# laprade117/interactive-unet

Measured on AMD Instinct MI355X. Metric: voxels/sec (train step + full-volume predict) on 128^3 chunks, higher is better.
Workload: dtype bf16

## Files before the change

interactive-unet_amd/csrc/common.h:

```cpp
#pragma once
#include <hip/hip_runtime.h>
#include <stdint.h>
#include <cstdio>
#include <cstdlib>
#include <type_traits>
#include "../../include/iunet.h"
#include "launchers.h"

typedef _Float16 f16;
typedef __bf16 bf16;
typedef _Float16 f16x8 __attribute__((ext_vector_type(8)));
typedef _Float16 f16x4 __attribute__((ext_vector_type(4)));
typedef _Float16 f16x2 __attribute__((ext_vector_type(2)));
typedef __bf16 bf16x8 __attribute__((ext_vector_type(8)));
typedef float f32x4 __attribute__((ext_vector_type(4)));
typedef unsigned int u32x4 __attribute__((ext_vector_type(4)));

struct TView {
  void* ptr;
  long long sample_stride;
  int planes;
};

template <typename T> struct Vec8;
// ... 262 lines not shown
  a = __builtin_amdgcn_cvt_pk_fp8_f32(c[2], c[3], a, true);
  int b = __builtin_amdgcn_cvt_pk_fp8_f32(c[4], c[5], 0, false);
  b = __builtin_amdgcn_cvt_pk_fp8_f32(c[6], c[7], b, true);
  return u32x2_t{(unsigned)a, (unsigned)b};
}
__device__ __forceinline__ u32x2_t x2m_hi8(const f16x8 hi);
template <bool CLAMPED = false>
__device__ __forceinline__ void x2m_split8(const float (&r)[8], f16x8& hi, f16x8& lo, u32x2_t& lo8, u32x2_t& hi8) {
  typedef short s16x2 __attribute__((ext_vector_type(2)));
  float res[8];
#pragma unroll
  for (int j = 0; j < 8; ++j) {
    const float v = CLAMPED ? r[j] : fminf(fmaxf(r[j], -65504.f), 65504.f);
    const f16 h = (f16)v;
    res[j] = v - (float)h;
    hi[j] = h; lo[j] = (f16)res[j];
  }
  s16x2 a = s16x2{0, 0}, b = s16x2{0, 0};
  a = __builtin_amdgcn_cvt_scalef32_pk_fp8_f32(a, res[0], res[1], 0.0625f, false);
  a = __builtin_amdgcn_cvt_scalef32_pk_fp8_f32(a, res[2], res[3], 0.0625f, true);
  b = __builtin_amdgcn_cvt_scalef32_pk_fp8_f32(b, res[4], res[5], 0.0625f, false);
  b = __builtin_amdgcn_cvt_scalef32_pk_fp8_f32(b, res[6], res[7], 0.0625f, true);
  lo8 = u32x2_t{__builtin_bit_cast(unsigned, a), __builtin_bit_cast(unsigned, b)};
  hi8 = x2m_hi8(hi);
}
__device__ __forceinline__ float x2_load_in(const void* p, long long off, int dt) {
  switch (dt) {
    case 0: return ((const float*)p)[off];
    case 1: return (float)((const f16*)p)[off];
    case 2: return __fdiv_rn((float)((const unsigned char*)p)[off], 255.0f);
    default: return (float)((const bf16*)p)[off];
  }
}
__device__ __forceinline__ void x2m_pool_keys(const f16x8 hi, const u32x2_t lo8, unsigned (&k)[8]) {
  const u32x4 hb = __builtin_bit_cast(u32x4, hi);
  unsigned hf[4], lf[2];
#pragma unroll
  for (int d = 0; d < 4; ++d) hf[d] = hb[d] ^ (((hb[d] >> 15) & 0x00010001u) * 0x7fffu + 0x80008000u);
#pragma unroll
  for (int e = 0; e < 2; ++e) {
    const unsigned t = (lo8[e] >> 7) & 0x01010101u;
    lf[e] = lo8[e] ^ (((t << 7) - t) + 0x80808080u);
  }
#pragma unroll
  for (int j = 0; j < 8; ++j)
    k[j] = __builtin_amdgcn_perm(hf[j >> 1], lf[j >> 2], 0x0c000000u | ((5u + 2u * (j & 1)) << 16) | ((4u + 2u * (j & 1)) << 8) | (unsigned)(j & 3));
}
__device__ __forceinline__ void x2m_pool_unkeys(const unsigned (&k)[8], f16x8& hi, u32x2_t& lo8) {
  u32x4 hb;
#pragma unroll
  for (int d = 0; d < 4; ++d) {
    const unsigned f = __builtin_amdgcn_perm(k[2 * d + 1], k[2 * d], 0x06050201u);
    hb[d] = f ^ (0xffffffffu - ((f >> 15) & 0x00010001u) * 0x7fffu);
  }
#pragma unroll
  for (int e = 0; e < 2; ++e) {
    const unsigned t0 = __builtin_amdgcn_perm(k[4 * e + 1], k[4 * e], 0x0c0c0400u), t1 = __builtin_amdgcn_perm(k[4 * e + 3], k[4 * e + 2], 0x0c0c0400u);
    const unsigned f = __builtin_amdgcn_perm(t1, t0, 0x05040100u);
    const unsigned t = (f >> 7) & 0x01010101u;
    lo8[e] = f ^ (0xffffffffu - ((t << 7) - t));
  }
  hi = __builtin_bit_cast(f16x8, hb);
}
__device__ __forceinline__ unsigned lane_xor1(unsigned v) {
  return (unsigned)__builtin_amdgcn_update_dpp(0, (int)v, 0xB1, 0xF, 0xF, false);
}
// ... 37 lines not shown
```

interactive-unet_amd/csrc/loss_terms.h:

```cpp
#pragma once
#include "common.h"

namespace {

__device__ __forceinline__ float load_t(const void* p, long long off, int dt) {
  return dt == 0 ? ((const float*)p)[off] : (float)((const f16*)p)[off];
}

__device__ __forceinline__ float block_sum_256(float v, float* red ) {
  v = wave_sum(v);
  __syncthreads();
  if ((threadIdx.x & 63) == 0) red[threadIdx.x >> 6] = v;
  __syncthreads();
  return red[0] + red[1] + red[2] + red[3];
}

template <int NV>
__device__ __forceinline__ void block_reduce_store(const float (&vals)[NV], float* lds, float* out) {
  const int lane = threadIdx.x & 63, wave = threadIdx.x >> 6;
#pragma unroll
  for (int i = 0; i < NV; ++i) {
    const float v = wave_sum(vals[i]);
    if (lane == 0) lds[wave * NV + i] = v;
  }
  __syncthreads();
  for (int i = threadIdx.x; i < NV; i += 256) out[i] = lds[i] + lds[NV + i] + lds[2 * NV + i] + lds[3 * NV + i];
}

template <int NCLS>
__device__ __forceinline__ void loss_sums(const float (&l)[NCLS], const void* target, const void* weight, int tdtype, int n,
                                          long long vox, long long v, float (&acc)[NCLS][8]) {
  float mx = l[0];
#pragma unroll
  for (int c = 1; c < NCLS; ++c) mx = fmaxf(mx, l[c]);
  float e[NCLS], s = 0.f;
#pragma unroll
  for (int c = 0; c < NCLS; ++c) { e[c] = __expf(l[c] - mx); s += e[c]; }
  const float inv = 1.f / s;
#pragma unroll
  for (int c = 0; c < NCLS; ++c) {
    const float pr = e[c] * inv;
    const long long to = ((long long)n * NCLS + c) * vox + v;
    const float y = load_t(target, to, tdtype);
    const float w = weight ? load_t(weight, to, tdtype) : 1.f;
    const float ry = rintf(y), rp = rintf(pr);
    acc[c][0] += w; acc[c][1] += w * y; acc[c][2] += w * pr; acc[c][3] += w * y * pr;
    acc[c][4] += w * y * __logf(pr + 1e-12f);
    acc[c][5] += w * ry; acc[c][6] += w * rp; acc[c][7] += w * ry * rp;
  }
}

template <int NCLS>
__device__ __forceinline__ void loss_grad(const float (&l)[NCLS], const void* target, const void* weight, int tdtype, const float* coef,
                                          int n, long long vox, long long v, float lscale, float (&dl)[NCLS], float (&accb)[NCLS]) {
  float mx = l[0];
#pragma unroll
  for (int c = 1; c < NCLS; ++c) mx = fmaxf(mx, l[c]);
  float e[NCLS], s = 0.f;
#pragma unroll
  for (int c = 0; c < NCLS; ++c) { e[c] = __expf(l[c] - mx); s += e[c]; }
  const float inv = 1.f / s;
  float g[NCLS], dot = 0.f;
#pragma unroll
  for (int c = 0; c < NCLS; ++c) {
    const float pr = e[c] * inv;
    const long long to = ((long long)n * NCLS + c) * vox + v;
    const float y = load_t(target, to, tdtype);
    const float w = weight ? load_t(weight, to, tdtype) : 1.f;
    g[c] = w * (coef[c * 3] + coef[c * 3 + 1] * y) - coef[c * 3 + 2] * w * y / (pr + 1e-12f);
    e[c] = pr;
    dot += g[c] * pr;
  }
#pragma unroll
  for (int c = 0; c < NCLS; ++c) { dl[c] = e[c] * (g[c] - dot) * lscale; accb[c] += dl[c]; }
}

}
```

interactive-unet_amd/csrc/pointwise.hip:

```cpp
#include "common.h"
#include "head_out.h"

namespace {

struct FirstConvParams {
  const void* x;
  long long sN, sC, sD, sH, sW;
  int in_dtype;
  void* y; long long y_sstride;
  const void* w;
  const float* bias;
  float* stats;
  int N, D, H, W, Cin, Cout, nd, relu;
  int out8;
};

__device__ __forceinline__ float load_in(const void* p, long long off, int dt) {
  switch (dt) {
    case 0: return ((const float*)p)[off];
    case 1: return (float)((const f16*)p)[off];
    case 2: return (float)((const unsigned char*)p)[off] / 255.0f;
    default: return (float)((const bf16*)p)[off];
  }
}

template <typename T, int ND, int CIN>
__global__ __launch_bounds__(256) void first_conv_kernel(FirstConvParams p) {
  using V8 = typename Vec8<T>::type;
  constexpr int TZ = ND == 3 ? 4 : 1, TY = ND == 3 ? 8 : 16, TX = ND == 3 ? 16 : 32, PADZ = ND == 3 ? 1 : 0;
  constexpr int PZ = TZ + 2 * PADZ, PY = TY + 2, PX = TX + 2, NPIX = PZ * PY * PX;
  constexpr int TAPS = ND == 3 ? 27 : 9, KK = TAPS * CIN, KS = (KK + 31) / 32;
  constexpr int FX = TX / 16, NI = 8;
  __shared__ T xs[CIN * NPIX];
  __shared__ float red[4 * 4 * 8 * 2];
  const int tid = threadIdx.x, lane = tid & 63, wave = tid >> 6, l15 = lane & 15, q = lane >> 4;
  const int tilesZ = (p.D + TZ - 1) / TZ, tilesY = (p.H + TY - 1) / TY, tilesX = (p.W + TX - 1) / TX;
  const int tps = tilesZ * tilesY * tilesX;
  const int tile = blockIdx.x, n = tile / tps;
  int trem = tile - n * tps;
  const int tz_i = trem / (tilesY * tilesX);
  trem -= tz_i * tilesY * tilesX;
  const int ty_i = trem / tilesX, tx_i = trem - ty_i * tilesX;
  const int z0 = tz_i * TZ, y0 = ty_i * TY, x0 = tx_i * TX;
  const int cob = blockIdx.y;
  for (int it = tid; it < NPIX * CIN; it += 256) {
    const int c = it / NPIX, pix = it - c * NPIX;
    const int px = pix % PX, t2 = pix / PX, py = t2 % PY, pz = t2 / PY;
    const int gz = z0 + pz - PADZ, gy = y0 + py - 1, gx = x0 + px - 1;
    float v = 0.f;
    if ((unsigned)gz < (unsigned)p.D && (unsigned)gy < (unsigned)p.H && (unsigned)gx < (unsigned)p.W)
      v = load_in(p.x, n * p.sN + c * p.sC + gz * p.sD + gy * p.sH + gx * p.sW, p.in_dtype);
    xs[it] = from_f32<T>(v);
  }
  V8 a[KS][2];
  const V8* wp = (const V8*)p.w + (long long)cob * KS * 2 * 64 + lane;
#pragma unroll
  for (int ks = 0; ks < KS; ++ks) { a[ks][0] = wp[(ks * 2 + 0) * 64]; a[ks][1] = wp[(ks * 2 + 1) * 64]; }
  int koff[KS][8];
#pragma unroll
  for (int ks = 0; ks < KS; ++ks)
#pragma unroll
    for (int j = 0; j < 8; ++j) {
      const int k = 32 * ks + 8 * q + j;
      const int kc = k < KK ? k : 0;
      const int tap = kc / CIN, c = kc % CIN;
      const int dz = ND == 3 ? tap / 9 : 0, dy = (tap / 3) % 3, dx = tap % 3;
      koff[ks][j] = c * NPIX + (dz * PY + dy) * PX + dx;
    }
  __syncthreads();
  T* yout = (T*)p.y + (long long)n * p.y_sstride;
  const long long plane_stride = (long long)p.D * p.H * p.W * 8;
  float bias[8], s_sum[8], s_sq[8];
#pragma unroll
  for (int j = 0; j < 8; ++j) { bias[j] = p.bias ? p.bias[cob * 32 + 8 * q + j] : 0.f; s_sum[j] = 0.f; s_sq[j] = 0.f; }
#pragma unroll
  for (int nf = 0; nf < NI; ++nf) {
    const int f = wave * NI + nf;
    const int xh = f % FX, row = f / FX, fy = row % TY, fz = row / TY;
    const int base = (fz * PY + fy) * PX + xh * 16 + l15;
    f32x4 acc0 = f32x4{0, 0, 0, 0}, acc1 = f32x4{0, 0, 0, 0};
#pragma unroll
    for (int ks = 0; ks < KS; ++ks) {
      V8 b;
#pragma unroll
      for (int j = 0; j < 8; ++j) b[j] = xs[base + koff[ks][j]];
      acc0 = mfma16<T>(a[ks][0], b, acc0);
      acc1 = mfma16<T>(a[ks][1], b, acc1);
    }
    const int gz = z0 + fz, gy = y0 + fy, gx = x0 + xh * 16 + l15;
    const bool ok = gz < p.D && gy < p.H && gx < p.W;
    float vals[8];
#pragma unroll
    for (int j = 0; j < 4; ++j) { vals[j] = acc0[j]; vals[4 + j] = acc1[j]; }
    if (p.stats && ok) {
#pragma unroll
      for (int j = 0; j < 8; ++j) { s_sum[j] += vals[j]; s_sq[j] += vals[j] * vals[j]; }
    }
    V8 o;
#pragma unroll
    for (int j = 0; j < 8; ++j) {
      float r = vals[j] + bias[j];
      if (p.relu) r = fmaxf(r, 0.f);
      o[j] = from_f32<T>(r);
    }
    if (ok) {
      if (!p.out8) *(V8*)(yout + (long long)(cob * 4 + q) * plane_stride + (((long long)gz * p.H + gy) * p.W + gx) * 8) = o;
      else e4m3_store8<T>((unsigned char*)p.y + (long long)n * p.y_sstride, cob * 4 + q, ((long long)gz * p.H + gy) * p.W + gx,
// ... 685 lines not shown
```

interactive-unet_amd/csrc/train_misc.hip:

```cpp
#include "common.h"

namespace {


struct ConvTDgradParams {
  const void* dy; long long dy_ss;
  void* dx; long long dx_ss;
  const void* wpk;
  int N, D, H, W, Cin, Cout;
};

template <typename T, int ND>
__global__ __launch_bounds__(256) void convT_dgrad_kernel(ConvTDgradParams p) {
  using V8 = V8T<T>;
  constexpr int NPOS = ND == 3 ? 8 : 4;
  const int lane = threadIdx.x & 63, wave = threadIdx.x >> 6;
  const int l15 = lane & 15, q = lane >> 4;
  const int xg = (p.W + 15) / 16;
  const long long rows = (long long)p.D * p.H * xg;
  const long long wid = (long long)blockIdx.x * 4 + wave;
  if (wid >= rows * p.N) return;
  const int n = (int)(wid / rows);
  const long long r = wid - n * rows;
  const int xb = (int)(r % xg), y = (int)((r / xg) % p.H), z = (int)(r / ((long long)xg * p.H));
// ... 305 lines not shown
  const long long per_b4 = (long long)Cin * Cout * npos / 4;
  const int col4 = threadIdx.x & 15, grp = threadIdx.x >> 4;
  const long long j4 = (long long)blockIdx.x * 16 + col4;
  const f32x4* slab4 = (const f32x4*)slab;
  f32x4 s = f32x4{0.f, 0.f, 0.f, 0.f};
  for (int b = grp; b < nb; b += 16) s += slab4[b * per_b4 + j4];
  red[grp][col4] = s;
  __syncthreads();
  if (grp != 0) return;
#pragma unroll
  for (int g = 1; g < 16; ++g) s += red[g][col4];
  const int ncob = Cout / 32;
#pragma unroll
  for (int k = 0; k < 4; ++k) {
    const long long j = j4 * 4 + k;
    const int c = (int)(j & 31), r = (int)((j >> 5) & 31);
    long long t = j >> 10;
    const int pos = (int)(t % npos); t /= npos;
    const int cob = (int)(t % ncob), cib = (int)(t / ncob);
    dW[((long long)(cib * 32 + r) * Cout + cob * 32 + c) * npos + pos] = s[k];
  }
}

struct FirstWgradParams {
  const void* x; long long sN, sC, sD, sH, sW; int in_dtype;
  const void* dy; long long dy_ss;
  const void* yraw; long long y_ss;
  const float* mean; const float* invstd; const float* coef; const float* scale; const float* shift;
  float* slab;
  int N, D, H, W, Cin, Cout;
  int tilesZ, tilesY, tilesX;
};

__device__ __forceinline__ float load_in2(const void* p, long long off, int dt) {
  switch (dt) {
    case 0: return ((const float*)p)[off];
    case 1: return (float)((const f16*)p)[off];
    case 2: return (float)((const unsigned char*)p)[off] / 255.0f;
    default: return (float)((const bf16*)p)[off];
  }
}

template <typename T, int ND, int CIN>
__global__ __launch_bounds__(256, 2) void first_wgrad_kernel(FirstWgradParams p) {
  using V8 = V8T<T>;
  constexpr int TZ = ND == 3 ? 4 : 1, TY = ND == 3 ? 8 : 16, TX = ND == 3 ? 16 : 32, PADZ = ND == 3 ? 1 : 0;
  constexpr int PZ = TZ + 2 * PADZ, PY = TY + 2, PX = TX + 2, NPIX = PZ * PY * PX, NVOX = TZ * TY * TX;
  constexpr int TAPS = ND == 3 ? 27 : 9, KK = TAPS * CIN, NT = (KK + 15) / 16, KKP = NT * 16;
  constexpr int FX = TX / 16, NKS = NVOX / 32;
  constexpr int PLANE_Y = NVOX * 16 + 64;
  constexpr int XS_BYTES = ((CIN * NPIX * 2 + 255) / 256) * 256;
  extern __shared__ __attribute__((aligned(256))) unsigned char smem[];
  T* xs = (T*)smem;
  unsigned char* dys = smem + XS_BYTES;
  __shared__ __attribute__((aligned(16))) float par[7 * 32];
  if (p.yraw != nullptr && threadIdx.x < 7 * 32) {
    const int k = threadIdx.x >> 5, c = blockIdx.y * 32 + (threadIdx.x & 31);
    par[threadIdx.x] = k == 0 ? p.scale[c] : k == 1 ? p.shift[c] : k == 2 ? p.mean[c] : k == 3 ? p.invstd[c] : p.coef[c * 3 + (k - 4)];
  }
  const unsigned lds_y = (unsigned)(size_t)(__attribute__((address_space(3))) unsigned char*)dys;
  const int tid = threadIdx.x, lane = tid & 63;
  const int wave = __builtin_amdgcn_readfirstlane(tid >> 6);
  const int g = lane >> 4, i16 = lane & 15, q = i16 >> 2, pp = i16 & 3, gh = g >> 1, gl = g & 1;
  const int cob = blockIdx.y;
  const unsigned laneY = lds_y + (pp >> 1) * PLANE_Y + (pp & 1) * 8 + (gh * 16 + gl * 8 + q) * 16;
  int col_off[NT];
#pragma unroll
  for (int ct = 0; ct < NT; ++ct) {
    const int kk = ct * 16 + i16, kc = kk < KK ? kk : 0;
    const int tap = kc / CIN, c = kc % CIN;
    const int dz = ND == 3 ? tap / 9 : 0, dy_ = (tap / 3) % 3, dx = tap % 3;
    col_off[ct] = c * NPIX + (dz * PY + dy_) * PX + dx;
  }
  f32x4 acc[2][NT];
#pragma unroll
  for (int t = 0; t < 2; ++t)
#pragma unroll
    for (int ct = 0; ct < NT; ++ct) acc[t][ct] = f32x4{0, 0, 0, 0};
  const int tps = p.tilesZ * p.tilesY * p.tilesX, ntiles = tps * p.N;
  const long long plane = (long long)p.D * p.H * p.W * 8;
  constexpr int XIT = (NPIX * CIN + 255) / 256, YIT = NVOX * 4 / 256;
  float xr[XIT];
  u32x4 yr[YIT], yw[YIT];
  unsigned oky = 0;
  auto load_tile = [&](int tile) {
    oky = 0;
    const int n = tile / tps;
    int trem = tile - n * tps;
    const int tz_i = trem / (p.tilesY * p.tilesX);
    trem -= tz_i * p.tilesY * p.tilesX;
    const int ty_i = trem / p.tilesX, tx_i = trem - ty_i * p.tilesX;
    const int z0 = tz_i * TZ, y0 = ty_i * TY, x0 = tx_i * TX;
#pragma unroll
    for (int k = 0; k < XIT; ++k) {
      const int it = tid + k * 256;
      const int c = it / NPIX, pix = it - c * NPIX;
      const int px = pix % PX, t2 = pix / PX, py = t2 % PY, pz = t2 / PY;
      const int gz = z0 + pz - PADZ, gy = y0 + py - 1, gx = x0 + px - 1;
      float v = 0.f;
      if (it < NPIX * CIN && (unsigned)gz < (unsigned)p.D && (unsigned)gy < (unsigned)p.H && (unsigned)gx < (unsigned)p.W)
        v = load_in2(p.x, n * p.sN + c * p.sC + gz * p.sD + gy * p.sH + gx * p.sW, p.in_dtype);
      xr[k] = v;
    }
    const T* dyin = (const T*)p.dy + (long long)n * p.dy_ss + (long long)cob * 4 * plane;
#pragma unroll
    for (int it = 0; it < YIT; ++it) {
      const int idx = tid + it * 256, pl = idx / NVOX, pix = idx - pl * NVOX;
      const int px = pix % TX, t2 = pix / TX, py = t2 % TY, pz = t2 / TY;
      const int gz = z0 + pz, gy = y0 + py, gx = x0 + px;
      u32x4 v = u32x4{0u, 0u, 0u, 0u};
      if (gz < p.D && gy < p.H && gx < p.W) v = *(const u32x4*)(dyin + pl * plane + (((long long)gz * p.H + gy) * p.W + gx) * 8);
      yr[it] = v;
      oky |= (gz < p.D && gy < p.H && gx < p.W) ? (1u << it) : 0u;
      if (p.yraw != nullptr) {
        u32x4 w = u32x4{0u, 0u, 0u, 0u};
        if (gz < p.D && gy < p.H && gx < p.W)
          w = *(const u32x4*)((const T*)p.yraw + (long long)n * p.y_ss + (long long)(cob * 4 + pl) * plane + (((long long)gz * p.H + gy) * p.W + gx) * 8);
        yw[it] = w;
      }
    }
  };
  auto commit_tile = [&]() {
#pragma unroll
    for (int k = 0; k < XIT; ++k) {
      const int it = tid + k * 256;
      if (it < NPIX * CIN) xs[it] = from_f32<T>(xr[k]);
    }
#pragma unroll
    for (int it = 0; it < YIT; ++it) {
      const int idx = tid + it * 256, pl = idx / NVOX, pix = idx - pl * NVOX;
      u32x4 v = yr[it];
      if (p.yraw != nullptr && ((oky >> it) & 1u)) {
        const V8 g = __builtin_bit_cast(V8, v), yy = __builtin_bit_cast(V8, yw[it]);
        V8 o;
        const f32x4* pp = (const f32x4*)(par + pl * 8);
        float cs[7][8];
#pragma unroll
        for (int k = 0; k < 7; ++k) {
          const f32x4 lo = pp[k * 8], hi = pp[k * 8 + 1];
#pragma unroll
          for (int j = 0; j < 4; ++j) { cs[k][j] = lo[j]; cs[k][4 + j] = hi[j]; }
        }
#pragma unroll
        for (int j = 0; j < 8; ++j) {
          const float yv = to_f32<T>(yy[j]);
          const float zv = to_f32<T>(from_f32<T>(fmaf(cs[0][j], yv, cs[1][j])));
          const float d = zv > 0.f ? to_f32<T>(g[j]) : 0.f;
          const float xh = (yv - cs[2][j]) * cs[3][j];
          o[j] = from_f32<T>(cs[4][j] * (d - cs[5][j] - xh * cs[6][j]));
        }
        v = __builtin_bit_cast(u32x4, o);
      }
      *(u32x4*)(dys + pl * PLANE_Y + pix * 16) = v;
    }
  };
  if ((int)blockIdx.x < ntiles) load_tile(blockIdx.x);
  for (int tile = blockIdx.x; tile < ntiles; tile += gridDim.x) {
    __syncthreads();
    commit_tile();
    __syncthreads();
    if (tile + (int)gridDim.x < ntiles) load_tile(tile + gridDim.x);
    for (int ks = wave; ks < NKS; ks += 4) {
      const int f = 2 * ks + gh;
      const int xh = f % FX, row = f / FX, fy = row % TY, fz = row / TY;
      const int vbase = (fz * PY + fy) * PX + xh * 16 + gl * 8;
      const V8 a0 = tr_frag2<T>(laneY + (unsigned)(2 * ks * 256), 64);
      const V8 a1 = tr_frag2<T>(laneY + (unsigned)(2 * ks * 256) + 2 * PLANE_Y, 64);
#pragma unroll
      for (int ct = 0; ct < NT; ++ct) {
        V8 b;
#pragma unroll
        for (int j = 0; j < 8; ++j) b[j] = xs[vbase + j + col_off[ct]];
        acc[0][ct] = mfma16<T>(a0, b, acc[0][ct]);
        acc[1][ct] = mfma16<T>(a1, b, acc[1][ct]);
      }
    }
  }
  __syncthreads();
  float* red = (float*)smem;
#pragma unroll
  for (int t = 0; t < 2; ++t)
#pragma unroll
    for (int ct = 0; ct < NT; ++ct)
#pragma unroll
      for (int j = 0; j < 4; ++j) red[(wave * 32 + t * 16 + 4 * g + j) * KKP + ct * 16 + i16] = acc[t][ct][j];
  __syncthreads();
  float* slab = p.slab + ((long long)blockIdx.x * p.Cout + cob * 32) * KKP;
// ... 198 lines not shown
```

interactive-unet_amd/csrc/train_pointwise.hip:

```cpp
#include "common.h"
#include "loss_terms.h"

namespace {


__global__ __launch_bounds__(1024) void bn_finalize_kernel(const float* __restrict__ slab, int nparts, int C, double count,
                                                           const float* __restrict__ gamma, const float* __restrict__ beta,
                                                           float* running_mean, float* running_var, float momentum,
                                                           float eps, float* scale, float* shift, float* mean_o,
                                                           float* invstd_o) {
  const int c = blockIdx.x, nt = (int)blockDim.x, nw = nt >> 6;
  double s = 0.0, s2 = 0.0;
  for (int p = threadIdx.x; p < nparts; p += nt) {
    const float2 v = *(const float2*)(slab + ((long long)p * C + c) * 2);
    s += (double)v.x; s2 += (double)v.y;
  }
  __shared__ double red[2][16];
#pragma unroll
  for (int o = 32; o > 0; o >>= 1) { s += __shfl_xor(s, o); s2 += __shfl_xor(s2, o); }
  if ((threadIdx.x & 63) == 0) { red[0][threadIdx.x >> 6] = s; red[1][threadIdx.x >> 6] = s2; }
  __syncthreads();
  if (threadIdx.x == 0) {
    double g0[4], g1[4];
    for (int g = 0; g < nw / 4; ++g) {
// ... 447 lines not shown
      const float base = add_skip ? to_f32<T>(o[j]) : 0.f;
      o[j] = from_f32<T>(base + (best[j] == s ? to_f32<T>(g[j]) : 0.f));
    }
    *(V8T<T>*)(dz + n * dz_ss + off[s]) = o;
  }
}

struct HeadLossParams {
  const void* x; long long x_ss; int planes;
  const float* w; const float* bias;
  const void* target; const void* weight; int tdtype;
  float* slab;
  const float* coef;
  void* dx; long long dx_ss;
  float* dwslab;
  float loss_scale;
  const float* loss_scale_dev;
  int N; long long vox;
  const float* in_scale; const float* in_shift;
  int pss;
};

template <typename T>
__device__ __forceinline__ V8T<T> head_act(const HeadLossParams& p, V8T<T> v, int pl, int n) {
  if (p.in_scale == nullptr) return v;
  V8T<T> o;
#pragma unroll
  for (int j = 0; j < 8; ++j)
    o[j] = from_f32<T>(fmaxf(fmaf(p.in_scale[n * p.pss + pl * 8 + j], to_f32<T>(v[j]), p.in_shift[n * p.pss + pl * 8 + j]), 0.f));
  return o;
}

#define HEAD_FWD_ITER 8
template <typename T, int NCLS>
__global__ __launch_bounds__(256) void head_loss_fwd_kernel(HeadLossParams p) {
  const int n = blockIdx.y;
  float acc[NCLS][8];
#pragma unroll
  for (int c = 0; c < NCLS; ++c)
#pragma unroll
    for (int k = 0; k < 8; ++k) acc[c][k] = 0.f;
  for (int it = 0; it < HEAD_FWD_ITER; ++it) {
    const long long v = ((long long)blockIdx.x * HEAD_FWD_ITER + it) * 256 + threadIdx.x;
    if (v >= p.vox) break;
    const T* xin = (const T*)p.x + n * p.x_ss + v * 8;
    float l[NCLS];
#pragma unroll
    for (int c = 0; c < NCLS; ++c) l[c] = p.bias[c];
    for (int pl = 0; pl < p.planes; ++pl) {
      const V8T<T> xv = head_act<T>(p, *(const V8T<T>*)(xin + (long long)pl * p.vox * 8), pl, n);
#pragma unroll
      for (int j = 0; j < 8; ++j) {
        const float a = to_f32<T>(xv[j]);
#pragma unroll
        for (int c = 0; c < NCLS; ++c) l[c] = fmaf(a, p.w[c * p.planes * 8 + pl * 8 + j], l[c]);
      }
    }
    loss_sums<NCLS>(l, p.target, p.weight, p.tdtype, n, p.vox, v, acc);
  }
  __shared__ float red[4 * NCLS * 8];
  const long long part = (long long)n * gridDim.x + blockIdx.x;
  float vals[NCLS * 8];
#pragma unroll
  for (int c = 0; c < NCLS; ++c)
#pragma unroll
    for (int k = 0; k < 8; ++k) vals[c * 8 + k] = acc[c][k];
  block_reduce_store<NCLS * 8>(vals, red, p.slab + part * NCLS * 8);
}

__global__ __launch_bounds__(256) void loss_finalize_kernel(const float* __restrict__ slab, int nparts, int ncls, int kind,
                                                            int has_weight, double nvox_total, float* out ,
                                                            float* coef ) {
  __shared__ double sums[10][8];
  __shared__ double red[256];
  const int items = ncls * 8, groups = 256 / items, t = threadIdx.x;
  double s = 0.0;
  if (t < groups * items) {
    const long long total = (long long)nparts * items;
    long long e = t;
    for (; e + 3LL * groups * items < total; e += 4LL * groups * items) {
      const float a = slab[e], b = slab[e + (long long)groups * items], c = slab[e + 2LL * groups * items],
                  d = slab[e + 3LL * groups * items];
      s += (double)a; s += (double)b; s += (double)c; s += (double)d;
    }
    for (; e < total; e += (long long)groups * items) s += (double)slab[e];
  }
  red[t] = s;
  __syncthreads();
  if (t < items) {
    double a = 0.0;
    for (int g = 0; g < groups; ++g) a += red[g * items + t];
    sums[t >> 3][t & 7] = a;
  }
  __syncthreads();
  if (threadIdx.x != 0) return;
  const double eps = 1e-12;
  const bool use_ce = (kind == 0 || kind >= 4);
  const int base = kind >= 4 ? kind - 3 : kind;
  double loss = 0.0, dice_r = 0.0, iou_r = 0.0, mcc_r = 0.0;
  const double G = (double)ncls;
  for (int c = 0; c < ncls; ++c) {
    const double cnt = has_weight ? sums[c][0] : nvox_total;
    const double tp = sums[c][3] / cnt, fp = (sums[c][2] - sums[c][3]) / cnt, fn = (sums[c][1] - sums[c][3]) / cnt;
    const double tn = (sums[c][0] - sums[c][1] - sums[c][2] + sums[c][3]) / cnt;
    double s_tp = 0, s_tn = 0, s_fp = 0, s_fn = 0, score = 0;
    if (base == 1) {
      const double num = 2 * tp + eps, den = 2 * tp + fp + fn + eps;
      score = num / den; s_tp = (2 * den - 2 * num) / (den * den); s_fp = -num / (den * den); s_fn = s_fp;
    } else if (base == 2) {
      const double num = tp + eps, den = tp + fp + fn + eps;
      score = num / den; s_tp = (den - num) / (den * den); s_fp = -num / (den * den); s_fn = s_fp;
    } else if (base == 3) {
      const double a = tp + fp, b = tp + fn, cc = tn + fp, d = tn + fn;
      const double root = sqrt(a * b * cc * d), num = tp * tn - fp * fn + eps, den = root + eps;
      score = num / den;
      const double half = 0.5 / root;
      const double r_tp = half * (b * cc * d + a * cc * d), r_tn = half * (a * b * d + a * b * cc);
      const double r_fp = half * (b * cc * d + a * b * d), r_fn = half * (a * cc * d + a * b * cc);
      s_tp = (tn * den - num * r_tp) / (den * den); s_tn = (tp * den - num * r_tn) / (den * den);
      s_fp = (-fn * den - num * r_fp) / (den * den); s_fn = (-fp * den - num * r_fn) / (den * den);
    }
    if (base != 0) loss += (1.0 - score) / G;
    if (use_ce) loss += (-sums[c][4] / cnt) / G;
    const double k = -1.0 / (G * cnt);
    coef[c * 3 + 0] = (float)(k * (s_fp - s_tn));
    coef[c * 3 + 1] = (float)(k * ((s_tp - s_fn) - (s_fp - s_tn)));
// ... 543 lines not shown
    const float mn = b1 * mv + (1.f - b1) * gr;
    const float vn = b2 * vv + (1.f - b2) * gr * gr;
    mv = mn; vv = vn;
    const float denom = sqrtf(vn) / bc2_sqrt + eps;
    pn -= (lr / bc1) * (mn / denom);
    pv = pn;
  };
  const long long i = ((long long)blockIdx.x * 256 + threadIdx.x) * 4;
  if (i + 3 < n) {
    float4 pv = *(float4*)(p + i), mv = *(float4*)(m + i), vv = *(float4*)(v + i);
    const float4 gv = *(const float4*)(g + i);
    one(pv.x, gv.x, mv.x, vv.x); one(pv.y, gv.y, mv.y, vv.y); one(pv.z, gv.z, mv.z, vv.z); one(pv.w, gv.w, mv.w, vv.w);
    *(float4*)(p + i) = pv; *(float4*)(m + i) = mv; *(float4*)(v + i) = vv;
  } else {
    for (long long k = i; k < n; ++k) one(p[k], g[k], m[k], v[k]);
  }
}
__global__ void head_grad_scatter_kernel(const float* __restrict__ t, float* __restrict__ dw, float* __restrict__ db, int ncls, int C0) {
  const int i = blockIdx.x * blockDim.x + threadIdx.x;
  if (i < ncls * C0) {
    const int c = i / C0, ch = i - c * C0;
    dw[i] = t[((ch >> 3) * ncls + c) * 8 + (ch & 7)];
  } else if (i < ncls * C0 + ncls) {
    db[i - ncls * C0] = t[i];
  }
}

}

#define DT_OK(dt) IUNET_REQUIRE((dt) == 0 || (dt) == 1, "dtype must be 0 (f16) or 1 (bf16), got %d", (dt))

int iunet_loss_finalize_launch(const float* slab, int nparts, int ncls, int kind, int has_weight, double nvox_total, float* out4,
                               float* coef, hipStream_t stream) {
  hipLaunchKernelGGL(loss_finalize_kernel, dim3(1), dim3(256), 0, stream, slab, nparts, ncls, kind, has_weight, nvox_total, out4, coef);
  IUNET_CHECK_HIP(hipGetLastError());
  return IUNET_OK;
}

static const int BN_BWD_PER_BLOCK = 2048;
static const int BN_POOL_PER_BLOCK = 8192;
static int norm_pool_chunks(int nd, long long ovox) {
  const int per_block = BN_POOL_PER_BLOCK / (nd == 3 ? 8 : 4);
  return (int)((ovox + per_block - 1) / per_block);
}

static int norm_relu_fwd_launch(int dtype, const void* y, long long y_ss, void* z, long long z_ss, const void* scale, const void* shift, int C,
                                int N, long long vox, int pss, void* stream) {
  const dim3 grid((unsigned)((vox + 511) / 512), C / 8, N);
  iunet_dispatch(dtype, 2, false, [&](auto t, auto, auto) {
    using T = decltype(t);
    hipLaunchKernelGGL(bn_relu_fwd_kernel<T>, grid, dim3(256), 0, (hipStream_t)stream, (const T*)y, y_ss, (T*)z, z_ss, (const float*)scale,
                       (const float*)shift, C / 8, vox, pss);
  });
  IUNET_CHECK_HIP(hipGetLastError());
  return IUNET_OK;
}
static int norm_relu_pool_fwd_launch(int dtype, int nd, const void* y, long long y_ss, void* z, long long z_ss, void* pooled, long long p_ss,
                                     const void* scale, const void* shift, int C, int N, int Do, int Ho, int Wo, int pss, void* stream) {
  const long long ovox = (long long)Do * Ho * Wo;
  const dim3 grid((unsigned)((ovox + 255) / 256), C / 8, N);
  iunet_dispatch(dtype, nd, false, [&](auto t, auto ndc, auto) {
    using T = decltype(t);
    hipLaunchKernelGGL((bn_relu_pool_fwd_kernel<T, ndc.value>), grid, dim3(256), 0, (hipStream_t)stream, (const T*)y, y_ss, (T*)z, z_ss,
                       (T*)pooled, p_ss, (const float*)scale, (const float*)shift, Do, Ho, Wo, pss);
  });
  IUNET_CHECK_HIP(hipGetLastError());
  return IUNET_OK;
// ... 239 lines not shown

int iunet_head_loss_bwd_num_parts(int N, long long vox, int ncls, int C0) {
  const int iter = (C0 / 8) * ncls <= 16 ? 8 : HEAD_BWD_WIDE_ITER;
  return N * (int)((vox + 256LL * iter - 1) / (256LL * iter));
}

#define HEAD_SWITCH(KERN, TT)                                                                                   \
  switch (ncls) {                                                                                               \
    case 2: hipLaunchKernelGGL((KERN<TT, 2>), grid, dim3(256), 0, (hipStream_t)stream, p); break;               \
    case 3: hipLaunchKernelGGL((KERN<TT, 3>), grid, dim3(256), 0, (hipStream_t)stream, p); break;               \
    case 4: hipLaunchKernelGGL((KERN<TT, 4>), grid, dim3(256), 0, (hipStream_t)stream, p); break;               \
    case 5: hipLaunchKernelGGL((KERN<TT, 5>), grid, dim3(256), 0, (hipStream_t)stream, p); break;               \
    case 6: hipLaunchKernelGGL((KERN<TT, 6>), grid, dim3(256), 0, (hipStream_t)stream, p); break;               \
    case 7: hipLaunchKernelGGL((KERN<TT, 7>), grid, dim3(256), 0, (hipStream_t)stream, p); break;               \
    case 8: hipLaunchKernelGGL((KERN<TT, 8>), grid, dim3(256), 0, (hipStream_t)stream, p); break;               \
    case 9: hipLaunchKernelGGL((KERN<TT, 9>), grid, dim3(256), 0, (hipStream_t)stream, p); break;               \
    default: hipLaunchKernelGGL((KERN<TT, 10>), grid, dim3(256), 0, (hipStream_t)stream, p); break;             \
  }

static int head_loss_fwd_impl(int dtype, const void* x, long long x_ss, int C0, const void* w, const void* bias, int ncls,
                              const void* target, const void* weight, int tdtype, int kind, void* slab, void* out4, void* coef,
                              int N, long long vox, const void* in_scale, const void* in_shift, void* stream, int per_sample = 0) {
  DT_OK(dtype);
  IUNET_REQUIRE(x && w && bias && target && slab && out4 && coef, "head_loss_fwd: null pointer");
  IUNET_REQUIRE(ncls >= 2 && ncls <= 10, "head_loss: num_classes must be 2..10");
  IUNET_REQUIRE(kind >= 0 && kind <= 6, "head_loss: unknown loss kind %d", kind);
  IUNET_REQUIRE(tdtype == 0 || tdtype == 1, "head_loss: target dtype must be 0 (f32) or 1 (f16)");
  HeadLossParams p{};
  p.x = x; p.x_ss = x_ss; p.planes = C0 / 8; p.w = (const float*)w; p.bias = (const float*)bias;
  p.target = target; p.weight = weight; p.tdtype = tdtype; p.slab = (float*)slab; p.N = N; p.vox = vox;
  p.in_scale = (const float*)in_scale; p.in_shift = (const float*)in_shift; p.pss = per_sample ? C0 : 0;
  dim3 grid((unsigned)(iunet_head_loss_num_parts(N, vox) / N), N);
  if (dtype == 0) { HEAD_SWITCH(head_loss_fwd_kernel, f16) } else { HEAD_SWITCH(head_loss_fwd_kernel, bf16) }
  hipLaunchKernelGGL(loss_finalize_kernel, dim3(1), dim3(256), 0, (hipStream_t)stream, (const float*)slab,
                     iunet_head_loss_num_parts(N, vox), ncls, kind, weight != nullptr, (double)N * (double)vox,
                     (float*)out4, (float*)coef);
  IUNET_CHECK_HIP(hipGetLastError());
  return IUNET_OK;
}

int iunet_head_loss_fwd(int dtype, const void* x, long long x_ss, int C0, const void* w, const void* bias, int ncls,
                        const void* target, const void* weight, int tdtype, int kind, void* slab, void* out4, void* coef,
                        int N, long long vox, void* stream) {
  return head_loss_fwd_impl(dtype, x, x_ss, C0, w, bias, ncls, target, weight, tdtype, kind, slab, out4, coef, N, vox, nullptr, nullptr, stream);
}

int iunet_head_loss_fwd_act(int dtype, const void* x, long long x_ss, int C0, const void* w, const void* bias, int ncls,
                            const void* target, const void* weight, int tdtype, int kind, void* slab, void* out4, void* coef,
                            const void* in_scale, const void* in_shift, int N, long long vox, void* stream) {
  IUNET_REQUIRE(in_scale && in_shift, "head_loss_fwd_act: null scale / shift");
  return head_loss_fwd_impl(dtype, x, x_ss, C0, w, bias, ncls, target, weight, tdtype, kind, slab, out4, coef, N, vox, in_scale, in_shift, stream);
}

int iunet_head_loss_fwd_act_ps(int dtype, const void* x, long long x_ss, int C0, const void* w, const void* bias, int ncls,
                               const void* target, const void* weight, int tdtype, int kind, void* slab, void* out4, void* coef,
                               const void* in_scale, const void* in_shift, int per_sample, int N, long long vox, void* stream) {
  IUNET_REQUIRE(in_scale && in_shift, "head_loss_fwd_act: null scale / shift");
  return head_loss_fwd_impl(dtype, x, x_ss, C0, w, bias, ncls, target, weight, tdtype, kind, slab, out4, coef, N, vox, in_scale, in_shift, stream, per_sample);
}

static int head_loss_bwd_impl(int dtype, const void* x, long long x_ss, int C0, const void* w, const void* bias, int ncls,
                              const void* target, const void* weight, int tdtype, const void* coef, float loss_scale, void* dx,
                              long long dx_ss, void* dwslab, int N, long long vox, const void* in_scale, const void* in_shift,
                              void* stream, const void* loss_scale_dev = nullptr) {
  DT_OK(dtype);
  IUNET_REQUIRE(x && w && bias && target && coef && dx && dwslab, "head_loss_bwd: null pointer");
  IUNET_REQUIRE(ncls >= 2 && ncls <= 10, "head_loss: num_classes must be 2..10");
// ... 203 lines not shown
```

Measured before the change: 719.4 million.

## Batch global loads in first-conv staging, head loss, and loss finalize

Input staging in the first conv and first wgrad kernels now loads raw bits for several elements at once, with the dtype dispatch hoisted out of the loop, before converting and writing to shared memory. The wgrad kernel keeps per-channel BN coefficients in registers instead of shared memory and maps dy loads per wave. The head loss kernel loads targets up front and prefetches several activation planes before the FMA loop. The loss finalize kernel uses 1024 threads with a tree reduction. Together these aim to raise memory-level parallelism and cut serial latency, at the cost of more registers and possible occupancy loss.

```diff
diff --git a/interactive-unet_amd/csrc/common.h b/interactive-unet_amd/csrc/common.h
--- a/interactive-unet_amd/csrc/common.h
+++ b/interactive-unet_amd/csrc/common.h
@@ -318,6 +318,21 @@
     default: return (float)((const bf16*)p)[off];
   }
 }
+__device__ __forceinline__ unsigned load_in_bits(const void* p, long long off, int dt) {
+  switch (dt) {
+    case 0: return ((const unsigned*)p)[off];
+    case 2: return ((const unsigned char*)p)[off];
+    default: return ((const unsigned short*)p)[off];
+  }
+}
+__device__ __forceinline__ float in_bits_value(unsigned b, int dt) {
+  switch (dt) {
+    case 0: return __builtin_bit_cast(float, b);
+    case 1: return (float)__builtin_bit_cast(f16, (unsigned short)b);
+    case 2: return (float)(unsigned char)b / 255.0f;
+    default: return (float)__builtin_bit_cast(bf16, (unsigned short)b);
+  }
+}
 __device__ __forceinline__ void x2m_pool_keys(const f16x8 hi, const u32x2_t lo8, unsigned (&k)[8]) {
   const u32x4 hb = __builtin_bit_cast(u32x4, hi);
   unsigned hf[4], lf[2];
diff --git a/interactive-unet_amd/csrc/loss_terms.h b/interactive-unet_amd/csrc/loss_terms.h
--- a/interactive-unet_amd/csrc/loss_terms.h
+++ b/interactive-unet_amd/csrc/loss_terms.h
@@ -28,8 +28,28 @@
 }
 
 template <int NCLS>
-__device__ __forceinline__ void loss_sums(const float (&l)[NCLS], const void* target, const void* weight, int tdtype, int n,
-                                          long long vox, long long v, float (&acc)[NCLS][8]) {
+__device__ __forceinline__ void load_targets(const void* target, const void* weight, int tdtype, int n, long long vox, long long v,
+                                             float (&y)[NCLS], float (&w)[NCLS]) {
+  if (tdtype == 0) {
+#pragma unroll
+    for (int c = 0; c < NCLS; ++c) {
+      const long long to = ((long long)n * NCLS + c) * vox + v;
+      y[c] = ((const float*)target)[to]; w[c] = weight ? ((const float*)weight)[to] : 1.f;
+    }
+  } else {
+    f16 yh[NCLS], wh[NCLS];
+#pragma unroll
+    for (int c = 0; c < NCLS; ++c) {
+      const long long to = ((long long)n * NCLS + c) * vox + v;
+      yh[c] = ((const f16*)target)[to]; wh[c] = weight ? ((const f16*)weight)[to] : (f16)1.f;
+    }
+#pragma unroll
+    for (int c = 0; c < NCLS; ++c) { y[c] = (float)yh[c]; w[c] = (float)wh[c]; }
+  }
+}
+
+template <int NCLS>
+__device__ __forceinline__ void loss_sums(const float (&l)[NCLS], const float (&yv)[NCLS], const float (&wv)[NCLS], float (&acc)[NCLS][8]) {
   float mx = l[0];
 #pragma unroll
   for (int c = 1; c < NCLS; ++c) mx = fmaxf(mx, l[c]);
@@ -40,14 +60,20 @@
 #pragma unroll
   for (int c = 0; c < NCLS; ++c) {
     const float pr = e[c] * inv;
-    const long long to = ((long long)n * NCLS + c) * vox + v;
-    const float y = load_t(target, to, tdtype);
-    const float w = weight ? load_t(weight, to, tdtype) : 1.f;
+    const float y = yv[c], w = wv[c];
     const float ry = rintf(y), rp = rintf(pr);
     acc[c][0] += w; acc[c][1] += w * y; acc[c][2] += w * pr; acc[c][3] += w * y * pr;
     acc[c][4] += w * y * __logf(pr + 1e-12f);
     acc[c][5] += w * ry; acc[c][6] += w * rp; acc[c][7] += w * ry * rp;
   }
+}
+
+template <int NCLS>
+__device__ __forceinline__ void loss_sums(const float (&l)[NCLS], const void* target, const void* weight, int tdtype, int n,
+                                          long long vox, long long v, float (&acc)[NCLS][8]) {
+  float y[NCLS], w[NCLS];
+  load_targets<NCLS>(target, weight, tdtype, n, vox, v, y, w);
+  loss_sums<NCLS>(l, y, w, acc);
 }
 
 template <int NCLS>
diff --git a/interactive-unet_amd/csrc/pointwise.hip b/interactive-unet_amd/csrc/pointwise.hip
--- a/interactive-unet_amd/csrc/pointwise.hip
+++ b/interactive-unet_amd/csrc/pointwise.hip
@@ -14,15 +14,6 @@
   int N, D, H, W, Cin, Cout, nd, relu;
   int out8;
 };
-
-__device__ __forceinline__ float load_in(const void* p, long long off, int dt) {
-  switch (dt) {
-    case 0: return ((const float*)p)[off];
-    case 1: return (float)((const f16*)p)[off];
-    case 2: return (float)((const unsigned char*)p)[off] / 255.0f;
-    default: return (float)((const bf16*)p)[off];
-  }
-}
 
 template <typename T, int ND, int CIN>
 __global__ __launch_bounds__(256) void first_conv_kernel(FirstConvParams p) {
@@ -43,19 +34,40 @@
   const int ty_i = trem / tilesX, tx_i = trem - ty_i * tilesX;
   const int z0 = tz_i * TZ, y0 = ty_i * TY, x0 = tx_i * TX;
   const int cob = blockIdx.y;
-  for (int it = tid; it < NPIX * CIN; it += 256) {
-    const int c = it / NPIX, pix = it - c * NPIX;
-    const int px = pix % PX, t2 = pix / PX, py = t2 % PY, pz = t2 / PY;
-    const int gz = z0 + pz - PADZ, gy = y0 + py - 1, gx = x0 + px - 1;
-    float v = 0.f;
-    if ((unsigned)gz < (unsigned)p.D && (unsigned)gy < (unsigned)p.H && (unsigned)gx < (unsigned)p.W)
-      v = load_in(p.x, n * p.sN + c * p.sC + gz * p.sD + gy * p.sH + gx * p.sW, p.in_dtype);
-    xs[it] = from_f32<T>(v);
-  }
   V8 a[KS][2];
   const V8* wp = (const V8*)p.w + (long long)cob * KS * 2 * 64 + lane;
 #pragma unroll
   for (int ks = 0; ks < KS; ++ks) { a[ks][0] = wp[(ks * 2 + 0) * 64]; a[ks][1] = wp[(ks * 2 + 1) * 64]; }
+  float bias[8];
+#pragma unroll
+  for (int j = 0; j < 8; ++j) bias[j] = p.bias ? p.bias[cob * 32 + 8 * q + j] : 0.f;
+  constexpr int XIT = (NPIX * CIN + 255) / 256, XCH = XIT < 8 ? XIT : 8;
+  auto stage = [&](auto dt) {
+    for (int k0 = 0; k0 < XIT; k0 += XCH) {
+      unsigned v[XCH], inside = 0;
+#pragma unroll
+      for (int k = 0; k < XCH; ++k) {
+        const int it = tid + (k0 + k) * 256;
+        const int c = it / NPIX, pix = it - c * NPIX;
+        const int px = pix % PX, t2 = pix / PX, py = t2 % PY, pz = t2 / PY;
+        const int gz = z0 + pz - PADZ, gy = y0 + py - 1, gx = x0 + px - 1;
+        const bool ok = it < NPIX * CIN && (unsigned)gz < (unsigned)p.D && (unsigned)gy < (unsigned)p.H && (unsigned)gx < (unsigned)p.W;
+        v[k] = load_in_bits(p.x, ok ? n * p.sN + c * p.sC + gz * p.sD + gy * p.sH + gx * p.sW : 0, decltype(dt)::value);
+        inside |= ok ? 1u << k : 0u;
+      }
+#pragma unroll
+      for (int k = 0; k < XCH; ++k) {
+        const int it = tid + (k0 + k) * 256;
+        if (it < NPIX * CIN) xs[it] = from_f32<T>((inside >> k) & 1u ? in_bits_value(v[k], decltype(dt)::value) : 0.f);
+      }
+    }
+  };
+  switch (p.in_dtype) {
+    case 0: stage(std::integral_constant<int, 0>{}); break;
+    case 1: stage(std::integral_constant<int, 1>{}); break;
+    case 2: stage(std::integral_constant<int, 2>{}); break;
+    default: stage(std::integral_constant<int, 3>{}); break;
+  }
   int koff[KS][8];
 #pragma unroll
   for (int ks = 0; ks < KS; ++ks)
@@ -70,9 +82,9 @@
   __syncthreads();
   T* yout = (T*)p.y + (long long)n * p.y_sstride;
   const long long plane_stride = (long long)p.D * p.H * p.W * 8;
-  float bias[8], s_sum[8], s_sq[8];
-#pragma unroll
-  for (int j = 0; j < 8; ++j) { bias[j] = p.bias ? p.bias[cob * 32 + 8 * q + j] : 0.f; s_sum[j] = 0.f; s_sq[j] = 0.f; }
+  float s_sum[8], s_sq[8];
+#pragma unroll
+  for (int j = 0; j < 8; ++j) { s_sum[j] = 0.f; s_sq[j] = 0.f; }
 #pragma unroll
   for (int nf = 0; nf < NI; ++nf) {
     const int f = wave * NI + nf;
diff --git a/interactive-unet_amd/csrc/train_misc.hip b/interactive-unet_amd/csrc/train_misc.hip
--- a/interactive-unet_amd/csrc/train_misc.hip
+++ b/interactive-unet_amd/csrc/train_misc.hip
@@ -361,15 +361,6 @@
   int tilesZ, tilesY, tilesX;
 };
 
-__device__ __forceinline__ float load_in2(const void* p, long long off, int dt) {
-  switch (dt) {
-    case 0: return ((const float*)p)[off];
-    case 1: return (float)((const f16*)p)[off];
-    case 2: return (float)((const unsigned char*)p)[off] / 255.0f;
-    default: return (float)((const bf16*)p)[off];
-  }
-}
-
 template <typename T, int ND, int CIN>
 __global__ __launch_bounds__(256, 2) void first_wgrad_kernel(FirstWgradParams p) {
   using V8 = V8T<T>;
@@ -382,11 +373,6 @@
   extern __shared__ __attribute__((aligned(256))) unsigned char smem[];
   T* xs = (T*)smem;
   unsigned char* dys = smem + XS_BYTES;
-  __shared__ __attribute__((aligned(16))) float par[7 * 32];
-  if (p.yraw != nullptr && threadIdx.x < 7 * 32) {
-    const int k = threadIdx.x >> 5, c = blockIdx.y * 32 + (threadIdx.x & 31);
-    par[threadIdx.x] = k == 0 ? p.scale[c] : k == 1 ? p.shift[c] : k == 2 ? p.mean[c] : k == 3 ? p.invstd[c] : p.coef[c * 3 + (k - 4)];
-  }
   const unsigned lds_y = (unsigned)(size_t)(__attribute__((address_space(3))) unsigned char*)dys;
   const int tid = threadIdx.x, lane = tid & 63;
   const int wave = __builtin_amdgcn_readfirstlane(tid >> 6);
@@ -408,80 +394,89 @@
     for (int ct = 0; ct < NT; ++ct) acc[t][ct] = f32x4{0, 0, 0, 0};
   const int tps = p.tilesZ * p.tilesY * p.tilesX, ntiles = tps * p.N;
   const long long plane = (long long)p.D * p.H * p.W * 8;
-  constexpr int XIT = (NPIX * CIN + 255) / 256, YIT = NVOX * 4 / 256;
-  float xr[XIT];
+  float cs[7][8];
+  if (p.yraw != nullptr) {
+    const int c0 = cob * 32 + wave * 8;
+#pragma unroll
+    for (int j = 0; j < 8; ++j) {
+      cs[0][j] = p.scale[c0 + j]; cs[1][j] = p.shift[c0 + j]; cs[2][j] = p.mean[c0 + j]; cs[3][j] = p.invstd[c0 + j];
+      cs[4][j] = p.coef[(c0 + j) * 3]; cs[5][j] = p.coef[(c0 + j) * 3 + 1]; cs[6][j] = p.coef[(c0 + j) * 3 + 2];
+    }
+  }
+  constexpr int XIT = (NPIX * CIN + 255) / 256, YIT = NVOX / 64;
+  unsigned xr[XIT];
   u32x4 yr[YIT], yw[YIT];
-  unsigned oky = 0;
-  auto load_tile = [&](int tile) {
-    oky = 0;
-    const int n = tile / tps;
-    int trem = tile - n * tps;
+  unsigned oky = 0, okx = 0;
+  struct Origin { int n, z0, y0, x0; };
+  auto origin = [&](int tile) {
+    Origin o;
+    o.n = tile / tps;
+    int trem = tile - o.n * tps;
     const int tz_i = trem / (p.tilesY * p.tilesX);
     trem -= tz_i * p.tilesY * p.tilesX;
     const int ty_i = trem / p.tilesX, tx_i = trem - ty_i * p.tilesX;
-    const int z0 = tz_i * TZ, y0 = ty_i * TY, x0 = tx_i * TX;
-#pragma unroll
-    for (int k = 0; k < XIT; ++k) {
-      const int it = tid + k * 256;
-      const int c = it / NPIX, pix = it - c * NPIX;
-      const int px = pix % PX, t2 = pix / PX, py = t2 % PY, pz = t2 / PY;
-      const int gz = z0 + pz - PADZ, gy = y0 + py - 1, gx = x0 + px - 1;
-      float v = 0.f;
-      if (it < NPIX * CIN && (unsigned)gz < (unsigned)p.D && (unsigned)gy < (unsigned)p.H && (unsigned)gx < (unsigned)p.W)
-        v = load_in2(p.x, n * p.sN + c * p.sC + gz * p.sD + gy * p.sH + gx * p.sW, p.in_dtype);
-      xr[k] = v;
-    }
-    const T* dyin = (const T*)p.dy + (long long)n * p.dy_ss + (long long)cob * 4 * plane;
-#pragma unroll
-    for (int it = 0; it < YIT; ++it) {
-      const int idx = tid + it * 256, pl = idx / NVOX, pix = idx - pl * NVOX;
-      const int px = pix % TX, t2 = pix / TX, py = t2 % TY, pz = t2 / TY;
-      const int gz = z0 + pz, gy = y0 + py, gx = x0 + px;
-      u32x4 v = u32x4{0u, 0u, 0u, 0u};
-      if (gz < p.D && gy < p.H && gx < p.W) v = *(const u32x4*)(dyin + pl * plane + (((long long)gz * p.H + gy) * p.W + gx) * 8);
-      yr[it] = v;
-      oky |= (gz < p.D && gy < p.H && gx < p.W) ? (1u << it) : 0u;
-      if (p.yraw != nullptr) {
-        u32x4 w = u32x4{0u, 0u, 0u, 0u};
-        if (gz < p.D && gy < p.H && gx < p.W)
-          w = *(const u32x4*)((const T*)p.yraw + (long long)n * p.y_ss + (long long)(cob * 4 + pl) * plane + (((long long)gz * p.H + gy) * p.W + gx) * 8);
-        yw[it] = w;
+    o.z0 = tz_i * TZ; o.y0 = ty_i * TY; o.x0 = tx_i * TX;
+    return o;
+  };
+  auto load_x = [&](const Origin& o, int k) {
+    const int it = tid + k * 256;
+    const int c = it / NPIX, pix = it - c * NPIX;
+    const int px = pix % PX, t2 = pix / PX, py = t2 % PY, pz = t2 / PY;
+    const int gz = o.z0 + pz - PADZ, gy = o.y0 + py - 1, gx = o.x0 + px - 1;
+    const bool ok = it < NPIX * CIN && (unsigned)gz < (unsigned)p.D && (unsigned)gy < (unsigned)p.H && (unsigned)gx < (unsigned)p.W;
+    xr[k] = load_in_bits(p.x, ok ? o.n * p.sN + c * p.sC + gz * p.sD + gy * p.sH + gx * p.sW : 0, p.in_dtype);
+    okx |= ok ? 1u << k : 0u;
+  };
+  auto load_y = [&](const Origin& o, int it) {
+    const int pix = lane + it * 64;
+    const int px = pix % TX, t2 = pix / TX, py = t2 % TY, pz = t2 / TY;
+    const int gz = o.z0 + pz, gy = o.y0 + py, gx = o.x0 + px;
+    const bool ok = gz < p.D && gy < p.H && gx < p.W;
+    const long long off = (long long)(cob * 4 + wave) * plane + (((long long)gz * p.H + gy) * p.W + gx) * 8;
+    u32x4 v = u32x4{0u, 0u, 0u, 0u};
+    if (ok) v = *(const u32x4*)((const T*)p.dy + (long long)o.n * p.dy_ss + off);
+    yr[it] = v;
+    oky |= ok ? 1u << it : 0u;
+    if (p.yraw != nullptr) {
+      u32x4 w = u32x4{0u, 0u, 0u, 0u};
+      if (ok) w = *(const u32x4*)((const T*)p.yraw + (long long)o.n * p.y_ss + off);
+      yw[it] = w;
+    }
+  };
+  auto commit_x = [&](int k) {
+    const int it = tid + k * 256;
+    if (it < NPIX * CIN) xs[it] = from_f32<T>((okx >> k) & 1u ? in_bits_value(xr[k], p.in_dtype) : 0.f);
+  };
+  auto commit_y = [&](int it) {
+    u32x4 v = yr[it];
+    if (p.yraw != nullptr && ((oky >> it) & 1u)) {
+      const V8 g = __builtin_bit_cast(V8, v), yy = __builtin_bit_cast(V8, yw[it]);
+      V8 o;
+#pragma unroll
+      for (int j = 0; j < 8; ++j) {
+        const float yv = to_f32<T>(yy[j]);
+        const float zv = to_f32<T>(from_f32<T>(fmaf(cs[0][j], yv, cs[1][j])));
+        const float d = zv > 0.f ? to_f32<T>(g[j]) : 0.f;
+        const float xh = (yv - cs[2][j]) * cs[3][j];
+        o[j] = from_f32<T>(cs[4][j] * (d - cs[5][j] - xh * cs[6][j]));
       }
-    }
+      v = __builtin_bit_cast(u32x4, o);
+    }
+    *(u32x4*)(dys + wave * PLANE_Y + (lane + it * 64) * 16) = v;
+  };
+  auto load_tile = [&](int tile) {
+    const Origin o = origin(tile);
+    okx = oky = 0;
+#pragma unroll
+    for (int k = 0; k < XIT; ++k) load_x(o, k);
+#pragma unroll
+    for (int it = 0; it < YIT; ++it) load_y(o, it);
   };
   auto commit_tile = [&]() {
 #pragma unroll
-    for (int k = 0; k < XIT; ++k) {
-      const int it = tid + k * 256;
-      if (it < NPIX * CIN) xs[it] = from_f32<T>(xr[k]);
-    }
-#pragma unroll
-    for (int it = 0; it < YIT; ++it) {
-      const int idx = tid + it * 256, pl = idx / NVOX, pix = idx - pl * NVOX;
-      u32x4 v = yr[it];
-      if (p.yraw != nullptr && ((oky >> it) & 1u)) {
-        const V8 g = __builtin_bit_cast(V8, v), yy = __builtin_bit_cast(V8, yw[it]);
-        V8 o;
-        const f32x4* pp = (const f32x4*)(par + pl * 8);
-        float cs[7][8];
-#pragma unroll
-        for (int k = 0; k < 7; ++k) {
-          const f32x4 lo = pp[k * 8], hi = pp[k * 8 + 1];
-#pragma unroll
-          for (int j = 0; j < 4; ++j) { cs[k][j] = lo[j]; cs[k][4 + j] = hi[j]; }
-        }
-#pragma unroll
-        for (int j = 0; j < 8; ++j) {
-          const float yv = to_f32<T>(yy[j]);
-          const float zv = to_f32<T>(from_f32<T>(fmaf(cs[0][j], yv, cs[1][j])));
-          const float d = zv > 0.f ? to_f32<T>(g[j]) : 0.f;
-          const float xh = (yv - cs[2][j]) * cs[3][j];
-          o[j] = from_f32<T>(cs[4][j] * (d - cs[5][j] - xh * cs[6][j]));
-        }
-        v = __builtin_bit_cast(u32x4, o);
-      }
-      *(u32x4*)(dys + pl * PLANE_Y + pix * 16) = v;
-    }
+    for (int k = 0; k < XIT; ++k) commit_x(k);
+#pragma unroll
+    for (int it = 0; it < YIT; ++it) commit_y(it);
   };
   if ((int)blockIdx.x < ntiles) load_tile(blockIdx.x);
   for (int tile = blockIdx.x; tile < ntiles; tile += gridDim.x) {
diff --git a/interactive-unet_amd/csrc/train_pointwise.hip b/interactive-unet_amd/csrc/train_pointwise.hip
--- a/interactive-unet_amd/csrc/train_pointwise.hip
+++ b/interactive-unet_amd/csrc/train_pointwise.hip
@@ -503,6 +503,7 @@
 }
 
 #define HEAD_FWD_ITER 8
+#define HEAD_FWD_PF 4
 template <typename T, int NCLS>
 __global__ __launch_bounds__(256) void head_loss_fwd_kernel(HeadLossParams p) {
   const int n = blockIdx.y;
@@ -515,19 +516,29 @@
     const long long v = ((long long)blockIdx.x * HEAD_FWD_ITER + it) * 256 + threadIdx.x;
     if (v >= p.vox) break;
     const T* xin = (const T*)p.x + n * p.x_ss + v * 8;
-    float l[NCLS];
+    float l[NCLS], yt[NCLS], wt[NCLS];
 #pragma unroll
     for (int c = 0; c < NCLS; ++c) l[c] = p.bias[c];
-    for (int pl = 0; pl < p.planes; ++pl) {
-      const V8T<T> xv = head_act<T>(p, *(const V8T<T>*)(xin + (long long)pl * p.vox * 8), pl, n);
-#pragma unroll
-      for (int j = 0; j < 8; ++j) {
-        const float a = to_f32<T>(xv[j]);
-#pragma unroll
-        for (int c = 0; c < NCLS; ++c) l[c] = fmaf(a, p.w[c * p.planes * 8 + pl * 8 + j], l[c]);
+    load_targets<NCLS>(p.target, p.weight, p.tdtype, n, p.vox, v, yt, wt);
+    for (int pl0 = 0; pl0 < p.planes; pl0 += HEAD_FWD_PF) {
+      V8T<T> xr[HEAD_FWD_PF];
+#pragma unroll
+      for (int i = 0; i < HEAD_FWD_PF; ++i)
+        if (pl0 + i < p.planes) xr[i] = *(const V8T<T>*)(xin + (long long)(pl0 + i) * p.vox * 8);
+#pragma unroll
+      for (int i = 0; i < HEAD_FWD_PF; ++i) {
+        const int pl = pl0 + i;
+        if (pl >= p.planes) break;
+        const V8T<T> xv = head_act<T>(p, xr[i], pl, n);
+#pragma unroll
+        for (int j = 0; j < 8; ++j) {
+          const float a = to_f32<T>(xv[j]);
+#pragma unroll
+          for (int c = 0; c < NCLS; ++c) l[c] = fmaf(a, p.w[c * p.planes * 8 + pl * 8 + j], l[c]);
+        }
       }
     }
-    loss_sums<NCLS>(l, p.target, p.weight, p.tdtype, n, p.vox, v, acc);
+    loss_sums<NCLS>(l, yt, wt, acc);
   }
   __shared__ float red[4 * NCLS * 8];
   const long long part = (long long)n * gridDim.x + blockIdx.x;
@@ -539,30 +550,35 @@
   block_reduce_store<NCLS * 8>(vals, red, p.slab + part * NCLS * 8);
 }
 
-__global__ __launch_bounds__(256) void loss_finalize_kernel(const float* __restrict__ slab, int nparts, int ncls, int kind,
+#define LOSS_FIN_THREADS 1024
+__global__ __launch_bounds__(LOSS_FIN_THREADS) void loss_finalize_kernel(const float* __restrict__ slab, int nparts, int ncls, int kind,
                                                             int has_weight, double nvox_total, float* out ,
                                                             float* coef ) {
   __shared__ double sums[10][8];
-  __shared__ double red[256];
-  const int items = ncls * 8, groups = 256 / items, t = threadIdx.x;
+  __shared__ double red[LOSS_FIN_THREADS];
+  const int items = ncls * 8, groups = LOSS_FIN_THREADS / items, t = threadIdx.x;
   double s = 0.0;
   if (t < groups * items) {
-    const long long total = (long long)nparts * items;
+    const long long total = (long long)nparts * items, step = (long long)groups * items;
     long long e = t;
-    for (; e + 3LL * groups * items < total; e += 4LL * groups * items) {
-      const float a = slab[e], b = slab[e + (long long)groups * items], c = slab[e + 2LL * groups * items],
-                  d = slab[e + 3LL * groups * items];
-      s += (double)a; s += (double)b; s += (double)c; s += (double)d;
-    }
-    for (; e < total; e += (long long)groups * items) s += (double)slab[e];
+    for (; e + 7 * step < total; e += 8 * step) {
+      float a[8];
+#pragma unroll
+      for (int k = 0; k < 8; ++k) a[k] = slab[e + k * step];
+#pragma unroll
+      for (int k = 0; k < 8; ++k) s += (double)a[k];
+    }
+    for (; e < total; e += step) s += (double)slab[e];
   }
   red[t] = s;
   __syncthreads();
-  if (t < items) {
-    double a = 0.0;
-    for (int g = 0; g < groups; ++g) a += red[g * items + t];
-    sums[t >> 3][t & 7] = a;
-  }
+  for (int n = groups; n > 1;) {
+    const int h = (n + 1) / 2;
+    if (t < (n - h) * items) red[t] += red[t + h * items];
+    __syncthreads();
+    n = h;
+  }
+  if (t < items) sums[t >> 3][t & 7] = red[t];
   __syncthreads();
   if (threadIdx.x != 0) return;
   const double eps = 1e-12;
@@ -1172,7 +1188,7 @@
 
 int iunet_loss_finalize_launch(const float* slab, int nparts, int ncls, int kind, int has_weight, double nvox_total, float* out4,
                                float* coef, hipStream_t stream) {
-  hipLaunchKernelGGL(loss_finalize_kernel, dim3(1), dim3(256), 0, stream, slab, nparts, ncls, kind, has_weight, nvox_total, out4, coef);
+  hipLaunchKernelGGL(loss_finalize_kernel, dim3(1), dim3(LOSS_FIN_THREADS), 0, stream, slab, nparts, ncls, kind, has_weight, nvox_total, out4, coef);
   IUNET_CHECK_HIP(hipGetLastError());
   return IUNET_OK;
 }
@@ -1478,7 +1494,7 @@
   p.in_scale = (const float*)in_scale; p.in_shift = (const float*)in_shift; p.pss = per_sample ? C0 : 0;
   dim3 grid((unsigned)(iunet_head_loss_num_parts(N, vox) / N), N);
   if (dtype == 0) { HEAD_SWITCH(head_loss_fwd_kernel, f16) } else { HEAD_SWITCH(head_loss_fwd_kernel, bf16) }
-  hipLaunchKernelGGL(loss_finalize_kernel, dim3(1), dim3(256), 0, (hipStream_t)stream, (const float*)slab,
+  hipLaunchKernelGGL(loss_finalize_kernel, dim3(1), dim3(LOSS_FIN_THREADS), 0, (hipStream_t)stream, (const float*)slab,
                      iunet_head_loss_num_parts(N, vox), ncls, kind, weight != nullptr, (double)N * (double)vox,
                      (float*)out4, (float*)coef);
   IUNET_CHECK_HIP(hipGetLastError());
```

Result: no change. 718.7 million (-0.1%).
